# rookieCookies/gpu-fluid-simulation

Hardware: AMD Instinct MI355X
Metric: M particle-steps/s (higher is better)
Workload: dtype f32; 1 GPU; dam_break_2d_16M; particles=16777216, scene=SURVEY.md §8d dam_break_2d, sort=bitonic, ref_quirks=True, parallelism=1 GPU, window=steps 5..54 from the lattice (--full: alt_windows for later regimes)

## Files before the change

gpu-fluid-simulation_amd/csrc/fs_neighbours.h:

```cpp
#pragma once
#include "fs_device.h"

namespace fsd {

#define FS_BLOCK 256

__device__ __forceinline__ uint32_t quirk_lo_fix(const StepParams& P, const u64* __restrict__ pairs,
                                                 const uint32_t* __restrict__ cs,
                                                 const uint32_t* __restrict__ start_ref) {
    if (!P.ref_quirks) return 0u;
    const uint32_t cmin = (uint32_t)(pairs[0] >> 32);
    if (cmin >= P.ncell) return 0u;
    const uint32_t v = start_ref[cmin];
    const uint32_t cnt = cs[cmin + 1];
    return v < cnt ? v : cnt;
}

__device__ __forceinline__ bool row_range(const StepParams& P, const uint32_t* __restrict__ cs, uint32_t cx,
                                          uint32_t y, uint32_t lo_fix, uint32_t* lo, uint32_t* hi) {
    if (y >= P.grid_v) return false;
    const uint32_t id_lo = y * P.grid_u + cx - 1u;
    if (id_lo >= P.ncell) return false;
    uint32_t id_hi = id_lo + 3u;
    if (id_hi > P.ncell) id_hi = P.ncell;
    uint32_t a = cs[id_lo];
    const uint32_t b = cs[id_hi];
    if (a == 0u) a = lo_fix;
    *lo = a;
    *hi = b;
    return a < b;
}

__device__ __forceinline__ RowRanges lane_row_ranges(const StepParams& P, const uint32_t* cs, uint32_t lo_fix, uint32_t cx,
                                                     uint32_t cy, bool live) {
    RowRanges R;
#pragma unroll
    for (int r = 0; r < 3; ++r) {
        R.lo[r] = 0; R.hi[r] = 0;
        if (live) (void)row_range(P, cs, cx, cy + (uint32_t)(r - 1), lo_fix, &R.lo[r], &R.hi[r]);
        if (R.hi[r] < R.lo[r]) R.hi[r] = R.lo[r];
    }
    return R;
}

#define NB_TILE 640
#ifndef NBF_TILE
#define NBF_TILE 544
#endif

__device__ __forceinline__ void store_block_bounds(const StepParams& P, uint32_t blk, const uint32_t* blo, const uint32_t* bhi) {
    uint32_t* bb = P.block_bounds + 8u * blk;
    bb[0] = blo[0]; bb[1] = blo[1]; bb[2] = blo[2]; bb[3] = bhi[0]; bb[4] = bhi[1]; bb[5] = bhi[2];
}
__device__ __forceinline__ void load_block_bounds(const StepParams& P, uint32_t blk, uint32_t* blo, uint32_t* bhi) {
    const uint32_t* bb = P.block_bounds + 8u * blk;
    blo[0] = bb[0]; blo[1] = bb[1]; blo[2] = bb[2]; bhi[0] = bb[3]; bhi[1] = bb[4]; bhi[2] = bb[5];
}

struct AosParticle { float2 position, predicted, velocity; float density; uint32_t grid; };

}
```

gpu-fluid-simulation_amd/csrc/kernels_density.hip:

```cpp
#include <stdlib.h>

#include "fs_force_lists.h"
#include "fs_kernels.h"
#include "fs_neighbours.h"

namespace fsd {

static_assert(FS_BLOCK == 256, "fs_force_lists.h lays the lists out for blocks of 256 particles");

__device__ __forceinline__ float density_cube_tol(float h2, float2 me, float2 q, float acc) {
    const float dx = q.x - me.x, dy = q.y - me.y;
    const float t = fmaxf(h2 - __builtin_fmaf(dx, dx, dy * dy), 0.0f);
    return __builtin_fmaf(t * t, t, acc);
}

template <bool MASS1 = false>
__device__ __forceinline__ float density_term(const StepParams& P, float h2, float2 me, float2 q) {
    const float dx = q.x - me.x, dy = q.y - me.y;
    const float r2 = dx * dx + dy * dy;
    float kern = 0.0f;
    if (!(r2 > h2)) {
        const float diff = h2 - r2;
        kern = P.poly6_norm * diff * diff * diff;
    }
    return MASS1 ? kern : P.mass * kern * 1.0f;
}

template <bool TOL, bool MASS1>
__device__ __forceinline__ void density_block(const StepParams& P, uint32_t blk, uint32_t n, const float2* __restrict__ pred,
                                              const uint32_t* __restrict__ cs, const uint32_t* __restrict__ start_ref,
                                              const u64* __restrict__ pairs, const unsigned long long* __restrict__ safe,
                                              float* __restrict__ rho_out, float2* __restrict__ rho2_out,
                                              uint32_t* __restrict__ force_defer, uint32_t* __restrict__ force_work,
                                              uint32_t* __restrict__ force_count, float2 (*s_pred)[NB_TILE], uint32_t* s_red) {
    const uint32_t i = blk * FS_BLOCK + threadIdx.x;
    const bool live = i < n;
    const uint32_t lo_fix = quirk_lo_fix(P, pairs, cs, start_ref);
    const float2 me = pred[live ? i : n - 1];
    uint32_t cx, cy;
    int32_t cg;
    uv_local(P, me, &cx, &cy, &cg);
    const float h2 = P.h * P.h;
    const RowRanges R = lane_row_ranges(P, cs, lo_fix, cx, cy, live);
    uint32_t blo[3], bhi[3];
    const bool fit = block_tile_bounds(R, s_red, blo, bhi, NB_TILE);
    if (P.block_bounds && threadIdx.x == 0) store_block_bounds(P, blk, blo, bhi);
    {
        const bool unfit = bhi[0] - blo[0] > NBF_TILE || bhi[1] - blo[1] > NBF_TILE || bhi[2] - blo[2] > NBF_TILE;
        const bool long_row = R.hi[0] - R.lo[0] > 32u || R.hi[1] - R.lo[1] > 32u || R.hi[2] - R.lo[2] > 32u;
        if ((unfit || __any(long_row)) && __builtin_amdgcn_ballot_w64(live) != 0 && (threadIdx.x & 63u) == 0u) {
            force_list_push(force_defer, force_work, force_count, P.n, blk, threadIdx.x >> 6, FS_LIST_PRE);
        }
    }
    float rho = 0.0f;
    if (fit) {
#pragma unroll
        for (int r = 0; r < 3; ++r)
            for (uint32_t j = threadIdx.x; j < bhi[r] - blo[r]; j += FS_BLOCK) s_pred[r][j] = pred[blo[r] + j];
        __syncthreads();
#pragma unroll
        for (int r = 0; r < 3; ++r) {
            const float2* sp = s_pred[r] - 0;
            const bool any = R.lo[r] < R.hi[r];
            const uint32_t hi = any ? R.hi[r] - blo[r] : 0u;
            uint32_t k = any ? R.lo[r] - blo[r] : 0u;
            if (TOL) {
                for (; k + 4u <= hi; k += 4u) {
                    const float2 q0 = sp[k], q1 = sp[k + 1u], q2 = sp[k + 2u], q3 = sp[k + 3u];
                    rho = density_cube_tol(h2, me, q0, rho); rho = density_cube_tol(h2, me, q1, rho);
                    rho = density_cube_tol(h2, me, q2, rho); rho = density_cube_tol(h2, me, q3, rho);
                }
                for (; k < hi; ++k) rho = density_cube_tol(h2, me, sp[k], rho);
                continue;
            }
            for (; k + 4u <= hi; k += 4u) {
                const float t0 = density_term<MASS1>(P, h2, me, sp[k]);
                const float t1 = density_term<MASS1>(P, h2, me, sp[k + 1u]);
                const float t2 = density_term<MASS1>(P, h2, me, sp[k + 2u]);
                const float t3 = density_term<MASS1>(P, h2, me, sp[k + 3u]);
                rho += t0; rho += t1; rho += t2; rho += t3;
            }
            for (; k < hi; ++k) rho += density_term<MASS1>(P, h2, me, sp[k]);
        }
    } else {
#pragma unroll
        for (int r = 0; r < 3; ++r)
            for (uint32_t k = R.lo[r]; k < R.hi[r]; ++k) {
                if (TOL) rho = density_cube_tol(h2, me, pred[k], rho);
                else rho += density_term<MASS1>(P, h2, me, pred[k]);
            }
    }
    if (!live) return;
    if (TOL) {
        rho = rho * (P.mass * P.poly6_norm);
        rho = fmaxf(fmaxf(rho, 1.19209290e-07f), 0.1f);
        rho_out[i] = rho;
        rho2_out[i] = make_float2(P.pressure_k * (rho - P.rest_density),
                                  (P.share_div && rho <= FS_RCP_HI) ? rcp_rn_fast(rho) : __fdiv_rn(1.0f, rho));
        return;
    }
    rho = fmaxf(rho, 1.19209290e-07f);
    rho = fmaxf(rho, 0.1f);
    if (rho_out) rho_out[i] = rho;
    const float press = P.pressure_k * (rho - P.rest_density);
    const bool ok = ((safe[i >> 6] >> (i & 63u)) & 1ull) != 0ull && rho <= FS_RCP_HI && fabsf(press) <= FS_PRESSURE_HI;
    const float y = (P.share_div && rho <= FS_RCP_HI) ? rcp_rn_fast(rho) : __fdiv_rn(1.0f, rho);
    rho2_out[i] = make_float2(rho, ok ? y : -y);
}

#define FS_DENSITY_ARGS                                                                                                   \
    StepParams P, const float2* __restrict__ pred, const uint32_t* __restrict__ cs, const uint32_t* __restrict__ start_ref, \
        const u64* __restrict__ pairs, const unsigned long long* __restrict__ safe, float* __restrict__ rho_out,         \
        float2* __restrict__ rho2_out, uint32_t* __restrict__ force_defer, uint32_t* __restrict__ force_work,            \
        uint32_t* __restrict__ force_count
template <bool TOL, bool MASS1>
__global__ __launch_bounds__(FS_BLOCK) void k_density(FS_DENSITY_ARGS) {
    __shared__ float2 s_pred[3][NB_TILE];
    __shared__ uint32_t s_red[24];
    const uint32_t n = P.n_live ? *P.n_live : P.n;
    uint32_t blk;
    if (!xcd_block(P, (n + FS_BLOCK - 1) / FS_BLOCK, &blk)) return;
    density_block<TOL, MASS1>(P, blk, n, pred, cs, start_ref, pairs, safe, rho_out, rho2_out, force_defer, force_work, force_count, s_pred, s_red);
}
template <bool TOL, bool MASS1>
__global__ __launch_bounds__(FS_BLOCK) void k_density_edge(FS_DENSITY_ARGS) {
    __shared__ float2 s_pred[3][NB_TILE];
    __shared__ uint32_t s_red[24];
    const uint32_t n = *P.n_live;
    const EdgeBlocks E = edge_blocks(P, cs, n, 1u);
    for (uint32_t t = blockIdx.x; t < edge_block_count(E); t += gridDim.x) {
        density_block<TOL, MASS1>(P, edge_block_at(E, t), n, pred, cs, start_ref, pairs, safe, rho_out, rho2_out, force_defer, force_work,
                           force_count, s_pred, s_red);
        __syncthreads();
    }
}

struct StConsts { float h2, cg, cl, sigma, tau; };

__device__ __forceinline__ void st_term(const StConsts& C, float2 me, float2 q, float w, float& nx, float& ny, float& L) {
    const float ox = q.x - me.x, oy = q.y - me.y;
    const float r2 = ox * ox + oy * oy;
    const bool in = !(r2 > C.h2);
    const float d = C.h2 - r2;
    const float k = (C.cg * d) * d;
    const float lk = (C.cl * d) * ((3.0f * r2) - C.h2);
    nx += in ? w * (k * ox) : 0.0f;
    ny += in ? w * (k * oy) : 0.0f;
    L += in ? w * lk : 0.0f;
}

template <bool MASS1>
__device__ __forceinline__ float st_weight(const StepParams& P, const float2* __restrict__ rho2, const float* __restrict__ rho_arr,
                                           uint32_t j) {
    if (MASS1) return fabsf(rho2[j].y);
    return __fdiv_rn(P.mass, rho_arr ? rho_arr[j] : rho2[j].x);
}

template <bool MASS1>
__global__ __launch_bounds__(FS_BLOCK) void k_surface_tension(StepParams P, StConsts C, const float2* __restrict__ pred,
                                                              const float2* __restrict__ rho2, const float* __restrict__ rho_arr,
                                                              const uint32_t* __restrict__ cs, const uint32_t* __restrict__ start_ref,
                                                              const u64* __restrict__ pairs, float2* __restrict__ st_out) {
    __shared__ float2 s_q[3][NB_TILE];
    __shared__ float s_w[3][NB_TILE];
    __shared__ uint32_t s_red[24];
    const uint32_t n = P.n;
    uint32_t blk;
    if (!xcd_block(P, (n + FS_BLOCK - 1) / FS_BLOCK, &blk)) return;
    const uint32_t i = blk * FS_BLOCK + threadIdx.x;
    const bool live = i < n;
    const uint32_t lo_fix = quirk_lo_fix(P, pairs, cs, start_ref);
    const float2 me = pred[live ? i : n - 1];
    uint32_t cx, cy;
    int32_t cg;
    uv_local(P, me, &cx, &cy, &cg);
    const RowRanges R = lane_row_ranges(P, cs, lo_fix, cx, cy, live);
    uint32_t blo[3], bhi[3];
    bool fit;
    if (P.block_bounds) {
        load_block_bounds(P, blk, blo, bhi);
        fit = bhi[0] - blo[0] <= NB_TILE && bhi[1] - blo[1] <= NB_TILE && bhi[2] - blo[2] <= NB_TILE;
    } else {
        fit = block_tile_bounds(R, s_red, blo, bhi, NB_TILE);
    }
    float nx = 0.0f, ny = 0.0f, L = 0.0f;
    if (fit) {
#pragma unroll
        for (int r = 0; r < 3; ++r)
            for (uint32_t j = threadIdx.x; j < bhi[r] - blo[r]; j += FS_BLOCK) {
                s_q[r][j] = pred[blo[r] + j];
                s_w[r][j] = st_weight<MASS1>(P, rho2, rho_arr, blo[r] + j);
            }
        __syncthreads();
#pragma unroll
        for (int r = 0; r < 3; ++r) {
            const bool any = R.lo[r] < R.hi[r];
            const uint32_t hi = any ? R.hi[r] - blo[r] : 0u;
            uint32_t k = any ? R.lo[r] - blo[r] : 0u;
            for (; k + 2u <= hi; k += 2u) {
                const float2 q0 = s_q[r][k], q1 = s_q[r][k + 1u];
                const float w0 = s_w[r][k], w1 = s_w[r][k + 1u];
                st_term(C, me, q0, w0, nx, ny, L);
                st_term(C, me, q1, w1, nx, ny, L);
            }
            if (k < hi) st_term(C, me, s_q[r][k], s_w[r][k], nx, ny, L);
        }
    } else {
#pragma unroll
        for (int r = 0; r < 3; ++r)
            for (uint32_t k = R.lo[r]; k < R.hi[r]; ++k) st_term(C, me, pred[k], st_weight<MASS1>(P, rho2, rho_arr, k), nx, ny, L);
    }
    if (!live) return;
    const float nl = sqrt_rn(nx * nx + ny * ny);
    float2 f = make_float2(0.0f, 0.0f);
    if (nl > C.tau && nl > 0.0f) {
        const float sc = __fdiv_rn(-C.sigma * L, nl);
        f = make_float2(sc * nx, sc * ny);
    }
    st_out[i] = f;
}

__device__ __forceinline__ float smoothstep_f(float a, float b, float x) {
    float t = __fdiv_rn(x - a, b - a);
    t = fminf(fmaxf(t, 0.0f), 1.0f);
    return t * t * (3.0f - 2.0f * t);
}

__global__ __launch_bounds__(FS_BLOCK) void k_render_density(StepParams P, float2 wmin, float2 wmax, uint32_t width,
                                                             uint32_t height, const float2* __restrict__ pred,
                                                             const float2* __restrict__ vel,
                                                             const uint32_t* __restrict__ cs,
                                                             const uint32_t* __restrict__ start_ref,
                                                             const u64* __restrict__ pairs, float4* __restrict__ out) {
    const uint32_t pix = blockIdx.x * FS_BLOCK + threadIdx.x;
    if (pix >= width * height) return;
    const uint32_t i = pix % width, j = pix / width;
    float2 pt;
    pt.x = wmin.x + __fdiv_rn((float)i + 0.5f, (float)width) * (wmax.x - wmin.x);
    pt.y = wmin.y + __fdiv_rn((float)j + 0.5f, (float)height) * (wmax.y - wmin.y);
    const uint32_t lo_fix = quirk_lo_fix(P, pairs, cs, start_ref);
    uint32_t cx, cy;
    xy_local(P, pt, &cx, &cy);
    float density = 0.0f, vfac = 0.0f;
    const float denom = P.sqr_radius / 2.0f;
    const uint32_t xlo = cx < 2u ? 0u : cx - 2u;
    const bool no_column = xlo >= P.grid_w;
    const uint32_t xhi = no_column ? xlo : (cx + 3u < P.grid_w ? cx + 3u : P.grid_w);
    for (int oy = -2; oy < 3; ++oy) {
        const uint32_t y = cy + (uint32_t)oy;
        if (y >= P.grid_h || no_column) continue;
        uint32_t a = cs[y * P.grid_w + xlo];
        const uint32_t b = cs[y * P.grid_w + xhi];
        if (a == 0u) a = lo_fix;
        for (uint32_t k = a; k < b; ++k) {
            const float2 q = pred[k];
            const float2 v = vel[k];
            const float ox = q.x - pt.x, oyv = q.y - pt.y;
            const float r2 = ox * ox + oyv * oyv;
            const float contrib = expf(__fdiv_rn(-r2, denom));
            density += contrib;
            vfac += contrib * sqrt_rn(v.x * v.x + v.y * v.y);
        }
    }
    vfac = vfac * 0.01f;
    vfac = __fdiv_rn(logf(1.0f + 5.0f * vfac), logf(1.0f + 5.0f));
    vfac = fminf(fmaxf(vfac, 0.0f), 1.0f);
    const float interior = smoothstep_f(0.5f, 1.5f, density);
    float edge = smoothstep_f(0.7f, 1.0f, density) - smoothstep_f(1.0f, 1.5f, density);
    edge = edge * (1.0f + vfac * 2.0f);
    const float br = (0.0f * (1.0f - vfac) + 1.0f * vfac) * interior;
    const float bg = (0.5f * (1.0f - vfac) + 0.0f * vfac) * interior;
    const float bb = (1.0f * (1.0f - vfac) + 0.0f * vfac) * interior;
    out[pix] = make_float4(br + edge, bg + edge, bb + edge, fminf(fmaxf(interior, 0.0f), 1.0f));
}

void launch_render_density(hipStream_t st, const StepParams& P_in, float2 wmin, float2 wmax, uint32_t width,
                           uint32_t height, const float2* pred, const float2* vel, const uint32_t* cs,
                           const uint32_t* start_ref, const u64* pairs, float4* out) {
    StepParams P = P_in;
    P.div_h.ok = 0;
    const uint32_t npix = width * height;
    hipLaunchKernelGGL(k_render_density, dim3((npix + FS_BLOCK - 1) / FS_BLOCK), dim3(FS_BLOCK), 0, st, P, wmin, wmax,
                       width, height, pred, vel, cs, start_ref, pairs, out);
}

void launch_density(hipStream_t st, const StepParams& P, const StepArrays& A, uint32_t edge_grid) {
    static const bool no_mass1 = getenv("FS_NO_MASS1") != nullptr;
    const bool tol = P.fast_math == 2, mass1 = P.mass == 1.0f && !tol && !no_mass1;
#define FS_LAUNCH_DENSITY(K, G)                                                                                        \
    do {                                                                                                               \
        if (tol) hipLaunchKernelGGL((K<true, false>), dim3(G), dim3(FS_BLOCK), 0, st, P, A.pred, A.cs, A.start_ref, A.pairs, A.safe, A.rho, A.rho2, A.fdefer, A.fwork, A.fcount); \
        else if (mass1) hipLaunchKernelGGL((K<false, true>), dim3(G), dim3(FS_BLOCK), 0, st, P, A.pred, A.cs, A.start_ref, A.pairs, A.safe, A.rho, A.rho2, A.fdefer, A.fwork, A.fcount); \
        else hipLaunchKernelGGL((K<false, false>), dim3(G), dim3(FS_BLOCK), 0, st, P, A.pred, A.cs, A.start_ref, A.pairs, A.safe, A.rho, A.rho2, A.fdefer, A.fwork, A.fcount); \
    } while (0)
    if (edge_grid) {
        FS_LAUNCH_DENSITY(k_density_edge, edge_grid);
        return;
    }
    const uint32_t nb = nblk(P.n), grid = xcd_grid(nb, P.xcd_chunk_log2);
    FS_LAUNCH_DENSITY(k_density, grid);
#undef FS_LAUNCH_DENSITY
}

void launch_surface_tension(hipStream_t st, const StepParams& P, const StepArrays& A, float sigma, float tau, float cg, float2* st_out) {
    if (P.n == 0) return;
    StConsts C;
    C.h2 = P.sqr_radius;
    C.cg = cg;
    C.cl = 2.0f * cg;
    C.sigma = sigma;
    C.tau = tau;
    const uint32_t grid = xcd_grid(nblk(P.n), P.xcd_chunk_log2);
    if (P.mass == 1.0f && !A.rho)
        hipLaunchKernelGGL(k_surface_tension<true>, dim3(grid), dim3(FS_BLOCK), 0, st, P, C, A.pred, A.rho2, A.rho, A.cs, A.start_ref, A.pairs, st_out);
    else
        hipLaunchKernelGGL(k_surface_tension<false>, dim3(grid), dim3(FS_BLOCK), 0, st, P, C, A.pred, A.rho2, A.rho, A.cs, A.start_ref, A.pairs, st_out);
}

}
```

gpu-fluid-simulation_amd/csrc/kernels_force.hip:

```cpp
#include <hip/hip_ext.h>

#include "fs_force_lists.h"
#include "fs_force_sweep.h"
#include "fs_kernels.h"

namespace fsd {

static_assert(FS_BLOCK == 256, "fs_force_lists.h lays the lists out for blocks of 256 particles");

template <int MODE, bool AOS, bool ST = false>
__device__ __forceinline__ void integrate_store(const StepParams& P, uint32_t i, const float2 me, const float2 mv, const float2 mrec,
                                                float mrho, const float2 p_own, const ForceAcc& A, uint32_t cx, uint32_t cy,
                                                const float2* __restrict__ tex, float2* __restrict__ pos_out,
                                                float2* __restrict__ vel_out, AosParticle* __restrict__ aos_out,
                                                const float* __restrict__ rho_arr, const float2* __restrict__ st_in) {
    const float fvx = A.fvx * P.visc_coeff;
    const float fvy = A.fvy * P.visc_coeff;

    float2 v = mv;
    float2 p = p_own;
    float ax = A.fpx + fvx, ay = A.fpy + fvy;
    if (ST) {
        const float2 fs = st_in[i];
        ax = ax + fs.x;
        ay = ay + fs.y;
    }
    if (MODE == 2) {
        v.x = __builtin_fmaf(ax * mrec.y, P.dt, v.x);
        v.y = __builtin_fmaf(ay * mrec.y, P.dt, v.y);
    } else {
        v.x += __fdiv_rn(ax, mrho) * P.dt;
        v.y += __fdiv_rn(ay, mrho) * P.dt;
    }
    v.x += P.gx * P.dt;
    v.y += P.gy * P.dt;
    if (P.mouse_state != 0) {
        const float dx = P.mouse_x - me.x, dy = P.mouse_y - me.y;
        const float dist = sqrt_rn(dx * dx + dy * dy);
        if (dist <= P.mouse_radius) {
            const float dirx = __fdiv_rn(__fdiv_rn(dx, dist), dist);
            const float diry = __fdiv_rn(__fdiv_rn(dy, dist), dist);
            const float ratio = __fdiv_rn(dist, P.mouse_radius);
            v.x += dirx * P.mouse_power * (float)P.mouse_state * ratio;
            v.y += diry * P.mouse_power * (float)P.mouse_state * ratio;
        }
    }
    if (!(v.x == v.x && v.y == v.y)) { v.x = 0.0f; v.y = 0.0f; }
    if (MODE == 2) {
        const float s2 = __builtin_fmaf(v.x, v.x, v.y * v.y);
        if (s2 > 250000.0f) { const float k = 500.0f * __builtin_amdgcn_rsqf(s2); v.x *= k; v.y *= k; }
    } else {
        const float s2 = v.x * v.x + v.y * v.y;
        if (s2 > 249000.0f) {
            const float speed = sqrt_rn(s2);
            if (speed > 500.0f) {
                v.x = __fdiv_rn(v.x, speed) * 500.0f;
                v.y = __fdiv_rn(v.y, speed) * 500.0f;
            }
        }
    }
    p.x += v.x * P.dt;
    p.y += v.y * P.dt;

    float2 force = make_float2(0.0f, 0.0f);
    if (!P.tex_zero) {
        const float uvx = (__fdiv_rn(me.x, P.bounds_x) * 1.0f) + 0.5f;
        const float uvy = (__fdiv_rn(me.y, P.bounds_y) * 1.0f) + 0.5f;
        const uint32_t px = f32_to_u32_sat(uvx * P.tex_w);
        const uint32_t py = f32_to_u32_sat(uvy * P.tex_h);
        const uint32_t tix = py * P.tex_w_u + px;
        if (tix < P.tex_len) force = tex[tix];
    }
    if (force.x != 0.0f || force.y != 0.0f) {
        const float p2wx = __fdiv_rn(P.bounds_x * 2.0f, P.tex_w);
        const float p2wy = __fdiv_rn(P.bounds_y * 2.0f, P.tex_h);
        const float fwx = force.x * p2wx, fwy = force.y * p2wy;
        const float len = sqrt_rn(force.x * force.x + force.y * force.y);
        const float nx = __fdiv_rn(force.x, len), ny = __fdiv_rn(force.y, len);
        p.x += fwx;
        p.y += fwy;
        const float vn = v.x * nx + v.y * ny;
        v.x -= (1.0f - P.damping) * vn * nx;
        v.y -= (1.0f - P.damping) * vn * ny;
    }
    if (fabsf(p.x) > P.bs_x) { p.x = P.bs_x * sign_f32(p.x); v.x *= -1.0f * P.damping; }
    if (fabsf(p.y) > P.bs_y) { p.y = P.bs_y * sign_f32(p.y); v.y *= -1.0f * P.damping; }
    pos_out[i] = p;
    vel_out[i] = v;
    if (AOS) {
        AosParticle a;
        a.position = p; a.predicted = me; a.velocity = v; a.density = MODE == 2 ? rho_arr[i] : mrho;
        a.grid = cy * P.grid_u + cx;
        aos_out[i] = a;
    }
}

#ifndef FS_FORCE_WAVES
#define FS_FORCE_WAVES 8
#endif
template <int MODE, bool AOS, bool GENERAL, bool ST>
__device__ __forceinline__ void force_block(const StepParams& P, uint32_t blk, uint32_t n, uint32_t wave_bits,
                                            const float2* __restrict__ pos_s, const float2* __restrict__ vel_s,
                                            const float2* __restrict__ pred, const float2* __restrict__ rho2,
                                            const uint32_t* __restrict__ cs, const uint32_t* __restrict__ start_ref,
                                            const u64* __restrict__ pairs, const float2* __restrict__ tex,
                                            float2* __restrict__ pos_out, float2* __restrict__ vel_out,
                                            AosParticle* __restrict__ aos_out, const float* __restrict__ rho_arr,
                                            uint32_t* __restrict__ defer_bits, uint32_t* __restrict__ worklist,
                                            uint32_t* __restrict__ work_count, const float2* __restrict__ st_in,
                                            float2 (*s_pred)[NBF_ROW], uint32_t* s_red) {
    const uint32_t tid = threadIdx.x;
    const uint32_t i = blk * FS_BLOCK + tid;
    bool live = i < n;
    if (GENERAL) live = live && ((wave_bits >> (tid >> 6)) & 1u);
    const bool pre = !GENERAL && ((wave_bits >> (tid >> 6)) & 1u);
    if (pre) live = false;
    const uint32_t ii = i < n ? i : n - 1;
    const uint32_t lo_fix = quirk_lo_fix(P, pairs, cs, start_ref);
    const float2 me = pred[ii];
    const float2 mv = vel_s[ii];
    const float2 mrec = rho2[ii];
    const float2 p_own = pos_s[P.pos_by_src ? (uint32_t)pairs[ii] : ii];
    const float mrho = MODE == 2 ? 0.0f : mrec.x;
    const bool me_ok = mrec.y > 0.0f;
    const float pressure = MODE == 2 ? mrec.x : P.pressure_k * (mrho - P.rest_density);
    ForceAcc A;
    A.fpx = A.fpy = A.fvx = A.fvy = 0.0f;
    A.seed = ii * 12u + P.frame_time * 69u;
    uint32_t cx, cy;
    int32_t cg;
    uv_local(P, me, &cx, &cy, &cg);
    if (P.n_live) {
        if (!slab_advances(P, cg)) live = false;
    }
    const RowRanges R = lane_row_ranges(P, cs, lo_fix, cx, cy, live);
    uint32_t blo[3], bhi[3];
    bool staged;
    if (P.block_bounds) {
        load_block_bounds(P, blk, blo, bhi);
        staged = bhi[0] - blo[0] <= NBF_TILE && bhi[1] - blo[1] <= NBF_TILE && bhi[2] - blo[2] <= NBF_TILE;
    } else {
        staged = block_tile_bounds(R, s_red, blo, bhi, NBF_TILE);
    }
    bool defer = !staged;
    if (staged) {
#pragma unroll
        for (int r = 0; r < 3; ++r)
            for (uint32_t j = tid; j < bhi[r] - blo[r]; j += FS_BLOCK) {
                s_pred[r][j] = pred[blo[r] + j];
            }
        __syncthreads();
        const bool long_row = R.hi[0] - R.lo[0] > 32u || R.hi[1] - R.lo[1] > 32u || R.hi[2] - R.lo[2] > 32u;
        if (!__any(long_row))
            defer = force_sweep_masks<MODE, GENERAL>(P, R, blo, ii, me, mv, pressure, vel_s, rho2, &s_pred[0][0], me_ok, A);
        else if (GENERAL)
            force_sweep_chunks<true, MODE>(P, R, blo, ii, me, mv, pressure, pred, vel_s, rho2, &s_pred[0][0], me_ok, A);
        else
            defer = true;
    } else if (GENERAL) {
        force_sweep_chunks<false, MODE>(P, R, blo, ii, me, mv, pressure, pred, vel_s, rho2, &s_pred[0][0], me_ok, A);
    }
    defer = __any(defer);
    if (!GENERAL && defer) {
        if (__builtin_amdgcn_ballot_w64(live) != 0 && (tid & 63u) == 0u) {
            force_list_push(defer_bits, worklist, work_count, P.n, blk, tid >> 6, FS_LIST_LATE);
        }
        return;
    }
    if (!live) return;
    integrate_store<MODE, AOS, ST>(P, i, me, mv, mrec, mrho, p_own, A, cx, cy, tex, pos_out, vel_out, aos_out, rho_arr, st_in);
}

__device__ __forceinline__ bool block_may_advance(const StepParams& P, const u64* __restrict__ pairs, uint32_t blk, uint32_t n) {
    if (!P.n_live || !P.transposed) return true;
    const uint32_t i0 = blk * FS_BLOCK;
    const uint32_t i1 = (i0 + FS_BLOCK < n ? i0 + FS_BLOCK : n) - 1u;
    const int32_t cf = (int32_t)((uint32_t)(pairs[i0] >> 32) / P.grid_u) + P.col_origin;
    const int32_t cl = (int32_t)((uint32_t)(pairs[i1] >> 32) / P.grid_u) + P.col_origin;
    if (P.adv_outside)
        return (cf < (int32_t)P.adv_lo && cl >= (int32_t)P.own_lo) || (cl >= (int32_t)P.adv_hi && cf < (int32_t)P.own_hi);
    return cl >= (int32_t)P.adv_lo && cf < (int32_t)P.adv_hi;
}

#define FS_FORCE_ARGS                                                                                                  \
    StepParams P, const float2* __restrict__ pos_s, const float2* __restrict__ vel_s, const float2* __restrict__ pred,  \
        const float2* __restrict__ rho2, const uint32_t* __restrict__ cs, const uint32_t* __restrict__ start_ref,       \
        const u64* __restrict__ pairs, const float2* __restrict__ tex, float2* __restrict__ pos_out,                   \
        float2* __restrict__ vel_out, AosParticle* __restrict__ aos_out, const float* __restrict__ rho_arr,            \
        uint32_t* __restrict__ defer_bits, uint32_t* __restrict__ worklist, uint32_t* __restrict__ work_count

template <int MODE, bool AOS, bool ST>
__global__ __launch_bounds__(FS_BLOCK) __attribute__((amdgpu_waves_per_eu(FS_FORCE_WAVES, FS_FORCE_WAVES))) void k_force(FS_FORCE_ARGS, uint32_t which, const float2* __restrict__ st_in) {
    __shared__ float2 s_pred[3][NBF_ROW];
    __shared__ uint32_t s_red[24];
    const uint32_t n = P.n_live ? *P.n_live : P.n;
    uint32_t blk;
    if (!xcd_block(P, (n + FS_BLOCK - 1) / FS_BLOCK, &blk)) return;
    if (!block_may_advance(P, pairs, blk, n)) return;
    force_block<MODE, AOS, false, ST>(P, blk, n, defer_bits[force_defer_word(blk, FS_LIST_PRE)], pos_s, vel_s, pred, rho2, cs, start_ref, pairs, tex,
                                      pos_out, vel_out, aos_out, rho_arr, defer_bits, worklist, work_count, st_in, s_pred, s_red);
}

template <int MODE, bool AOS, bool ST>
__global__ __launch_bounds__(FS_BLOCK) __attribute__((amdgpu_waves_per_eu(FS_FORCE_WAVES, FS_FORCE_WAVES))) void k_force_edge(FS_FORCE_ARGS, uint32_t which, const float2* __restrict__ st_in) {
    static_assert(!ST, "surface tension: single-domain handles only");
    __shared__ float2 s_pred[3][NBF_ROW];
    __shared__ uint32_t s_red[24];
    const uint32_t n = *P.n_live;
    const EdgeBlocks E = edge_blocks(P, cs, n, 0u);
    for (uint32_t t = blockIdx.x; t < edge_block_count(E); t += gridDim.x) {
        const uint32_t blk = edge_block_at(E, t);
        if (block_may_advance(P, pairs, blk, n))
            force_block<MODE, AOS, false, false>(P, blk, n, defer_bits[force_defer_word(blk, FS_LIST_PRE)], pos_s, vel_s, pred, rho2, cs, start_ref, pairs, tex,
                                                 pos_out, vel_out, aos_out, rho_arr, defer_bits, worklist, work_count, st_in, s_pred, s_red);
        __syncthreads();
    }
}

#ifndef FS_GENERAL_WAVES
#define FS_GENERAL_WAVES 5
#endif
template <int MODE, bool AOS, bool ST>
__global__ __launch_bounds__(FS_BLOCK) __attribute__((amdgpu_waves_per_eu(FS_GENERAL_WAVES, FS_GENERAL_WAVES))) void k_force_general(FS_FORCE_ARGS, uint32_t which, uint32_t* __restrict__ hint, const float2* __restrict__ st_in) {
    __shared__ float2 s_pred[3][NBF_ROW];
    __shared__ uint32_t s_red[24];
    const uint32_t n = P.n_live ? *P.n_live : P.n;
    if (hint && blockIdx.x == 0 && threadIdx.x == 0) *hint = which == 2u ? work_count[FS_LIST_PRE] + work_count[FS_LIST_LATE] : work_count[which];
    const uint32_t e_spread = force_list_spread();
    for (uint32_t w = (which == 2u ? 0u : which); w <= (which == 2u ? 1u : which); ++w) {
        const uint32_t count = work_count[w];
        const uint32_t* list = worklist + force_list_base(P.n, w);
        for (uint32_t e = count < gridDim.x ? e_spread : blockIdx.x; e < count; e += gridDim.x) {
            const uint32_t blk = list[e];
            if (!block_may_advance(P, pairs, blk, n)) continue;
            const uint32_t bits = defer_bits[force_defer_word(blk, w)];
            force_block<MODE, AOS, true, ST>(P, blk, n, bits, pos_s, vel_s, pred, rho2, cs, start_ref, pairs,
                                             tex, pos_out, vel_out, aos_out, rho_arr, defer_bits, worklist, work_count, st_in, s_pred,
                                             s_red);
            __syncthreads();
        }
    }
}

#include "kernels_force_quad.inc"

struct ForceArgs {
    StepParams P;
    const float2 *pos_s, *vel_s, *pred, *rho2;
    const uint32_t *cs, *start_ref;
    const u64* pairs;
    const float2* tex;
    float2 *pos_out, *vel_out;
    AosParticle* aos_out;
    const float* rho_arr;
    uint32_t *defer_bits, *worklist, *work_count;
};
template <typename K, typename... Own>
static void launch_force_kernel(K kernel, uint32_t grid, hipStream_t s, hipEvent_t stop_ev, const ForceArgs& a, Own... own) {
    hipExtLaunchKernelGGL(kernel, dim3(grid), dim3(FS_BLOCK), 0, s, nullptr, stop_ev, 0, a.P, a.pos_s, a.vel_s, a.pred, a.rho2, a.cs,
                          a.start_ref, a.pairs, a.tex, a.pos_out, a.vel_out, a.aos_out, a.rho_arr, a.defer_bits, a.worklist,
                          a.work_count, own...);
}

typedef void (*GeneralKernel)(FS_FORCE_ARGS, uint32_t, uint32_t*, const float2*);
typedef void (*LeanKernel)(FS_FORCE_ARGS, uint32_t, const float2*);
typedef void (*QuadKernel)(FS_FORCE_ARGS, uint32_t*, const float2*);

template <int MODE, bool ST> static GeneralKernel general_kernel(bool aos) { return aos ? k_force_general<MODE, true, ST> : k_force_general<MODE, false, ST>; }
template <bool ST> static GeneralKernel general_kernel(int mode, bool aos) {
    if (mode == 2) return general_kernel<2, ST>(aos);
    else if (mode == 1) return general_kernel<1, ST>(aos);
    else return general_kernel<0, ST>(aos);
}
static GeneralKernel general_kernel(int mode, bool aos, bool st) { return st ? general_kernel<true>(mode, aos) : general_kernel<false>(mode, aos); }

template <int MODE> static LeanKernel edge_kernel(bool aos) { return aos ? k_force_edge<MODE, true, false> : k_force_edge<MODE, false, false>; }
static LeanKernel edge_kernel(int mode, bool aos) {
    if (mode == 2) return edge_kernel<2>(aos);
    else if (mode == 1) return edge_kernel<1>(aos);
    else return edge_kernel<0>(aos);
}

template <int MODE, bool ST> static LeanKernel lean_kernel(bool aos) { return aos ? k_force<MODE, true, ST> : k_force<MODE, false, ST>; }
template <bool ST> static LeanKernel lean_kernel(int mode, bool aos) {
    if (mode == 2) return lean_kernel<2, ST>(aos);
    else if (mode == 1) return lean_kernel<1, ST>(aos);
    else return lean_kernel<0, ST>(aos);
}
static LeanKernel lean_kernel(int mode, bool aos, bool st) { return st ? lean_kernel<true>(mode, aos) : lean_kernel<false>(mode, aos); }

template <int MODE, bool ST> static QuadKernel quad_kernel(bool aos) { return aos ? k_force_quad<MODE, true, ST> : k_force_quad<MODE, false, ST>; }
template <bool ST> static QuadKernel quad_kernel(int mode, bool aos) { return mode == 1 ? quad_kernel<1, ST>(aos) : quad_kernel<0, ST>(aos); }
static QuadKernel quad_kernel(int mode, bool aos, bool st) { return st ? quad_kernel<true>(mode, aos) : quad_kernel<false>(mode, aos); }

#ifndef FS_GENERAL_GRID
#define FS_GENERAL_GRID 4080u
#endif
void launch_force(hipStream_t st, const StepParams& P, const StepArrays& A, const ForceLaunch& L) {
    const ForceArgs a = {P, A.pos_s, A.vel_s, A.pred, A.rho2, A.cs, A.start_ref, A.pairs, A.tex, A.pos_out, A.vel_out,
                         (AosParticle*)L.aos_out, A.rho, A.fdefer, A.fwork, A.fcount};
    const int mode = P.fast_math;
    const bool aos = L.aos_out != nullptr, surf = L.st_in != nullptr;
    const GeneralKernel general = general_kernel(mode, aos, surf);
    uint32_t* const no_hint = nullptr;
    const uint32_t nb = nblk(P.n), grid = xcd_grid(nb, P.xcd_chunk_log2);
    uint32_t gg = L.general_grid ? L.general_grid : FS_GENERAL_GRID;
    if (gg > nb) gg = nb;
    if (L.side) {
        (void)hipEventRecord(L.ev_fork, st);
        (void)hipStreamWaitEvent(L.side, L.ev_fork, 0);
        launch_force_kernel(general, gg, L.side, nullptr, a, FS_LIST_PRE, no_hint, L.st_in);
        (void)hipEventRecord(L.ev_join, L.side);
    }
    if (L.edge_grid) launch_force_kernel(edge_kernel(mode, aos), L.edge_grid, st, nullptr, a, 0u, L.st_in);
    else launch_force_kernel(lean_kernel(mode, aos, surf), grid, st, nullptr, a, 0u, L.st_in);
    if (L.side) {
        (void)hipStreamWaitEvent(st, L.ev_join, 0);
        launch_force_kernel(general, (nb < 256u ? nb : 256u), st, L.done, a, FS_LIST_LATE, no_hint, L.st_in);
    } else if (L.quad_entries != 0u && mode != 2 && (mode == 1 || P.share_div)) {
        uint32_t qg = 8u * L.quad_entries;
        qg = qg < 80u ? 80u : qg > 4080u ? 4080u : (qg + 39u) / 40u * 40u;
        launch_force_kernel(quad_kernel(mode, aos, surf), qg, st, nullptr, a, L.general_hint, L.st_in);
        launch_force_kernel(general, 240u, st, L.done, a, FS_LIST_LATE, no_hint, L.st_in);
    } else {
        launch_force_kernel(general, gg, st, L.done, a, 2u, L.general_hint, L.st_in);
    }
}
}
```

Baseline: 12720 M particle-steps/s.

## Issue neighbour-tile global loads into registers early before shared-memory staging

```diff
diff --git a/gpu-fluid-simulation_amd/csrc/fs_neighbours.h b/gpu-fluid-simulation_amd/csrc/fs_neighbours.h
--- a/gpu-fluid-simulation_amd/csrc/fs_neighbours.h
+++ b/gpu-fluid-simulation_amd/csrc/fs_neighbours.h
@@ -16,7 +16,7 @@
     return v < cnt ? v : cnt;
 }
 
-__device__ __forceinline__ bool row_range(const StepParams& P, const uint32_t* __restrict__ cs, uint32_t cx,
+__host__ __device__ __forceinline__ bool row_range(const StepParams& P, const uint32_t* __restrict__ cs, uint32_t cx,
                                           uint32_t y, uint32_t lo_fix, uint32_t* lo, uint32_t* hi) {
     if (y >= P.grid_v) return false;
     const uint32_t id_lo = y * P.grid_u + cx - 1u;
@@ -31,14 +31,28 @@
     return a < b;
 }
 
-__device__ __forceinline__ RowRanges lane_row_ranges(const StepParams& P, const uint32_t* cs, uint32_t lo_fix, uint32_t cx,
+__host__ __device__ __forceinline__ RowRanges lane_row_ranges(const StepParams& P, const uint32_t* cs, uint32_t lo_fix, uint32_t cx,
                                                      uint32_t cy, bool live) {
     RowRanges R;
+    bool ok[3];
+    uint32_t a[3], b[3];
 #pragma unroll
     for (int r = 0; r < 3; ++r) {
-        R.lo[r] = 0; R.hi[r] = 0;
-        if (live) (void)row_range(P, cs, cx, cy + (uint32_t)(r - 1), lo_fix, &R.lo[r], &R.hi[r]);
-        if (R.hi[r] < R.lo[r]) R.hi[r] = R.lo[r];
+        const uint32_t y = cy + (uint32_t)(r - 1);
+        const uint32_t id_lo = y * P.grid_u + cx - 1u;
+        ok[r] = live && y < P.grid_v && id_lo < P.ncell;
+        uint32_t id_hi = id_lo + 3u;
+        if (id_hi > P.ncell) id_hi = P.ncell;
+        a[r] = cs[ok[r] ? id_lo : 0u];
+        b[r] = cs[ok[r] ? id_hi : 0u];
+    }
+#pragma unroll
+    for (int r = 0; r < 3; ++r) {
+        uint32_t lo = a[r] == 0u ? lo_fix : a[r];
+        uint32_t hi = b[r];
+        if (!ok[r]) { lo = 0u; hi = 0u; }
+        R.lo[r] = lo;
+        R.hi[r] = hi < lo ? lo : hi;
     }
     return R;
 }
@@ -47,6 +61,32 @@
 #ifndef NBF_TILE
 #define NBF_TILE 544
 #endif
+
+#define FS_STAGE_TRIPS 3
+static_assert(NB_TILE <= FS_STAGE_TRIPS * FS_BLOCK && NBF_TILE <= FS_STAGE_TRIPS * FS_BLOCK,
+              "stage_rows_load / stage_rows_store cover a tile in FS_STAGE_TRIPS trips of the workgroup");
+template <typename T> struct StagedRows { T v[3][FS_STAGE_TRIPS]; };
+
+template <typename T, typename Fetch>
+__device__ __forceinline__ void stage_rows_load(StagedRows<T>& S, const uint32_t* blo, const uint32_t* bhi, Fetch fetch) {
+#pragma unroll
+    for (int r = 0; r < 3; ++r)
+#pragma unroll
+        for (int t = 0; t < FS_STAGE_TRIPS; ++t) {
+            const uint32_t j = threadIdx.x + (uint32_t)t * FS_BLOCK;
+            if (j < bhi[r] - blo[r]) S.v[r][t] = fetch(blo[r] + j);
+        }
+}
+template <typename T, typename Put>
+__device__ __forceinline__ void stage_rows_store(const StagedRows<T>& S, const uint32_t* blo, const uint32_t* bhi, Put put) {
+#pragma unroll
+    for (int r = 0; r < 3; ++r)
+#pragma unroll
+        for (int t = 0; t < FS_STAGE_TRIPS; ++t) {
+            const uint32_t j = threadIdx.x + (uint32_t)t * FS_BLOCK;
+            if (j < bhi[r] - blo[r]) put(r, j, S.v[r][t]);
+        }
+}
 
 __device__ __forceinline__ void store_block_bounds(const StepParams& P, uint32_t blk, const uint32_t* blo, const uint32_t* bhi) {
     uint32_t* bb = P.block_bounds + 8u * blk;
@@ -57,6 +97,11 @@
     blo[0] = bb[0]; blo[1] = bb[1]; blo[2] = bb[2]; bhi[0] = bb[3]; bhi[1] = bb[4]; bhi[2] = bb[5];
 }
 
+__device__ __forceinline__ bool recorded_tile_bounds(const StepParams& P, uint32_t blk, uint32_t* blo, uint32_t* bhi, uint32_t tile) {
+    load_block_bounds(P, blk, blo, bhi);
+    return bhi[0] - blo[0] <= tile && bhi[1] - blo[1] <= tile && bhi[2] - blo[2] <= tile;
+}
+
 struct AosParticle { float2 position, predicted, velocity; float density; uint32_t grid; };
 
 }
diff --git a/gpu-fluid-simulation_amd/csrc/kernels_density.hip b/gpu-fluid-simulation_amd/csrc/kernels_density.hip
--- a/gpu-fluid-simulation_amd/csrc/kernels_density.hip
+++ b/gpu-fluid-simulation_amd/csrc/kernels_density.hip
@@ -35,8 +35,8 @@
                                               uint32_t* __restrict__ force_count, float2 (*s_pred)[NB_TILE], uint32_t* s_red) {
     const uint32_t i = blk * FS_BLOCK + threadIdx.x;
     const bool live = i < n;
+    const float2 me = pred[live ? i : n - 1];
     const uint32_t lo_fix = quirk_lo_fix(P, pairs, cs, start_ref);
-    const float2 me = pred[live ? i : n - 1];
     uint32_t cx, cy;
     int32_t cg;
     uv_local(P, me, &cx, &cy, &cg);
@@ -54,9 +54,9 @@
     }
     float rho = 0.0f;
     if (fit) {
-#pragma unroll
-        for (int r = 0; r < 3; ++r)
-            for (uint32_t j = threadIdx.x; j < bhi[r] - blo[r]; j += FS_BLOCK) s_pred[r][j] = pred[blo[r] + j];
+        StagedRows<float2> S;
+        stage_rows_load(S, blo, bhi, [&](uint32_t k) { return pred[k]; });
+        stage_rows_store(S, blo, bhi, [&](int r, uint32_t j, float2 q) { s_pred[r][j] = q; });
         __syncthreads();
 #pragma unroll
         for (int r = 0; r < 3; ++r) {
@@ -150,11 +150,21 @@
 }
 
 template <bool MASS1>
+__device__ __forceinline__ float st_weight_operand(const float2* __restrict__ rho2, const float* __restrict__ rho_arr, uint32_t j) {
+    if (MASS1) return rho2[j].y;
+    return rho_arr ? rho_arr[j] : rho2[j].x;
+}
+template <bool MASS1>
+__device__ __forceinline__ float st_weight_of(const StepParams& P, float d) {
+    if (MASS1) return fabsf(d);
+    return __fdiv_rn(P.mass, d);
+}
+template <bool MASS1>
 __device__ __forceinline__ float st_weight(const StepParams& P, const float2* __restrict__ rho2, const float* __restrict__ rho_arr,
                                            uint32_t j) {
-    if (MASS1) return fabsf(rho2[j].y);
-    return __fdiv_rn(P.mass, rho_arr ? rho_arr[j] : rho2[j].x);
-}
+    return st_weight_of<MASS1>(P, st_weight_operand<MASS1>(rho2, rho_arr, j));
+}
+struct StCandidate { float2 q; float d; };
 
 template <bool MASS1>
 __global__ __launch_bounds__(FS_BLOCK) void k_surface_tension(StepParams P, StConsts C, const float2* __restrict__ pred,
@@ -178,19 +188,18 @@
     uint32_t blo[3], bhi[3];
     bool fit;
     if (P.block_bounds) {
-        load_block_bounds(P, blk, blo, bhi);
-        fit = bhi[0] - blo[0] <= NB_TILE && bhi[1] - blo[1] <= NB_TILE && bhi[2] - blo[2] <= NB_TILE;
+        fit = recorded_tile_bounds(P, blk, blo, bhi, NB_TILE);
     } else {
         fit = block_tile_bounds(R, s_red, blo, bhi, NB_TILE);
     }
     float nx = 0.0f, ny = 0.0f, L = 0.0f;
     if (fit) {
-#pragma unroll
-        for (int r = 0; r < 3; ++r)
-            for (uint32_t j = threadIdx.x; j < bhi[r] - blo[r]; j += FS_BLOCK) {
-                s_q[r][j] = pred[blo[r] + j];
-                s_w[r][j] = st_weight<MASS1>(P, rho2, rho_arr, blo[r] + j);
-            }
+        StagedRows<StCandidate> S;
+        stage_rows_load(S, blo, bhi, [&](uint32_t k) { return StCandidate{pred[k], st_weight_operand<MASS1>(rho2, rho_arr, k)}; });
+        stage_rows_store(S, blo, bhi, [&](int r, uint32_t j, const StCandidate& c) {
+            s_q[r][j] = c.q;
+            s_w[r][j] = st_weight_of<MASS1>(P, c.d);
+        });
         __syncthreads();
 #pragma unroll
         for (int r = 0; r < 3; ++r) {
diff --git a/gpu-fluid-simulation_amd/csrc/kernels_force.hip b/gpu-fluid-simulation_amd/csrc/kernels_force.hip
--- a/gpu-fluid-simulation_amd/csrc/kernels_force.hip
+++ b/gpu-fluid-simulation_amd/csrc/kernels_force.hip
@@ -1,4 +1,6 @@
 #include <hip/hip_ext.h>
+
+#include <type_traits>
 
 #include "fs_force_lists.h"
 #include "fs_force_sweep.h"
@@ -98,7 +100,12 @@
 #ifndef FS_FORCE_WAVES
 #define FS_FORCE_WAVES 8
 #endif
-template <int MODE, bool AOS, bool GENERAL, bool ST>
+struct NoStagedRows {};
+__device__ __forceinline__ void force_stage_load(StagedRows<float2>& S, const uint32_t* blo, const uint32_t* bhi,
+                                                 const float2* __restrict__ pred) {
+    stage_rows_load(S, blo, bhi, [&](uint32_t k) { return pred[k]; });
+}
+template <int MODE, bool AOS, bool GENERAL, bool ST, bool EARLY>
 __device__ __forceinline__ void force_block(const StepParams& P, uint32_t blk, uint32_t n, uint32_t wave_bits,
                                             const float2* __restrict__ pos_s, const float2* __restrict__ vel_s,
                                             const float2* __restrict__ pred, const float2* __restrict__ rho2,
@@ -116,11 +123,21 @@
     const bool pre = !GENERAL && ((wave_bits >> (tid >> 6)) & 1u);
     if (pre) live = false;
     const uint32_t ii = i < n ? i : n - 1;
-    const uint32_t lo_fix = quirk_lo_fix(P, pairs, cs, start_ref);
+    uint32_t blo[3], bhi[3];
+    bool staged = false;
+    std::conditional_t<EARLY, StagedRows<float2>, NoStagedRows> S;
+    const bool ahead = EARLY && P.block_bounds != nullptr;
+    if constexpr (EARLY) {
+        if (ahead) {
+            staged = recorded_tile_bounds(P, blk, blo, bhi, NBF_TILE);
+            if (staged) force_stage_load(S, blo, bhi, pred);
+        }
+    }
     const float2 me = pred[ii];
     const float2 mv = vel_s[ii];
     const float2 mrec = rho2[ii];
     const float2 p_own = pos_s[P.pos_by_src ? (uint32_t)pairs[ii] : ii];
+    const uint32_t lo_fix = quirk_lo_fix(P, pairs, cs, start_ref);
     const float mrho = MODE == 2 ? 0.0f : mrec.x;
     const bool me_ok = mrec.y > 0.0f;
     const float pressure = MODE == 2 ? mrec.x : P.pressure_k * (mrho - P.rest_density);
@@ -134,21 +151,22 @@
         if (!slab_advances(P, cg)) live = false;
     }
     const RowRanges R = lane_row_ranges(P, cs, lo_fix, cx, cy, live);
-    uint32_t blo[3], bhi[3];
-    bool staged;
-    if (P.block_bounds) {
-        load_block_bounds(P, blk, blo, bhi);
-        staged = bhi[0] - blo[0] <= NBF_TILE && bhi[1] - blo[1] <= NBF_TILE && bhi[2] - blo[2] <= NBF_TILE;
-    } else {
-        staged = block_tile_bounds(R, s_red, blo, bhi, NBF_TILE);
+    if (!ahead) {
+        if (P.block_bounds) staged = recorded_tile_bounds(P, blk, blo, bhi, NBF_TILE);
+        else staged = block_tile_bounds(R, s_red, blo, bhi, NBF_TILE);
+        if constexpr (EARLY) {
+            if (staged) force_stage_load(S, blo, bhi, pred);
+        }
     }
     bool defer = !staged;
     if (staged) {
+        if constexpr (EARLY) {
+            stage_rows_store(S, blo, bhi, [&](int r, uint32_t j, float2 q) { s_pred[r][j] = q; });
+        } else {
 #pragma unroll
-        for (int r = 0; r < 3; ++r)
-            for (uint32_t j = tid; j < bhi[r] - blo[r]; j += FS_BLOCK) {
-                s_pred[r][j] = pred[blo[r] + j];
-            }
+            for (int r = 0; r < 3; ++r)
+                for (uint32_t j = tid; j < bhi[r] - blo[r]; j += FS_BLOCK) s_pred[r][j] = pred[blo[r] + j];
+        }
         __syncthreads();
         const bool long_row = R.hi[0] - R.lo[0] > 32u || R.hi[1] - R.lo[1] > 32u || R.hi[2] - R.lo[2] > 32u;
         if (!__any(long_row))
@@ -197,7 +215,7 @@
     uint32_t blk;
     if (!xcd_block(P, (n + FS_BLOCK - 1) / FS_BLOCK, &blk)) return;
     if (!block_may_advance(P, pairs, blk, n)) return;
-    force_block<MODE, AOS, false, ST>(P, blk, n, defer_bits[force_defer_word(blk, FS_LIST_PRE)], pos_s, vel_s, pred, rho2, cs, start_ref, pairs, tex,
+    force_block<MODE, AOS, false, ST, true>(P, blk, n, defer_bits[force_defer_word(blk, FS_LIST_PRE)], pos_s, vel_s, pred, rho2, cs, start_ref, pairs, tex,
                                       pos_out, vel_out, aos_out, rho_arr, defer_bits, worklist, work_count, st_in, s_pred, s_red);
 }
 
@@ -211,7 +229,7 @@
     for (uint32_t t = blockIdx.x; t < edge_block_count(E); t += gridDim.x) {
         const uint32_t blk = edge_block_at(E, t);
         if (block_may_advance(P, pairs, blk, n))
-            force_block<MODE, AOS, false, false>(P, blk, n, defer_bits[force_defer_word(blk, FS_LIST_PRE)], pos_s, vel_s, pred, rho2, cs, start_ref, pairs, tex,
+            force_block<MODE, AOS, false, false, false>(P, blk, n, defer_bits[force_defer_word(blk, FS_LIST_PRE)], pos_s, vel_s, pred, rho2, cs, start_ref, pairs, tex,
                                                  pos_out, vel_out, aos_out, rho_arr, defer_bits, worklist, work_count, st_in, s_pred, s_red);
         __syncthreads();
     }
@@ -234,7 +252,7 @@
             const uint32_t blk = list[e];
             if (!block_may_advance(P, pairs, blk, n)) continue;
             const uint32_t bits = defer_bits[force_defer_word(blk, w)];
-            force_block<MODE, AOS, true, ST>(P, blk, n, bits, pos_s, vel_s, pred, rho2, cs, start_ref, pairs,
+            force_block<MODE, AOS, true, ST, false>(P, blk, n, bits, pos_s, vel_s, pred, rho2, cs, start_ref, pairs,
                                              tex, pos_out, vel_out, aos_out, rho_arr, defer_bits, worklist, work_count, st_in, s_pred,
                                              s_red);
             __syncthreads();
```

After: 13180 M particle-steps/s, median of 6. 1.04x the previous value.
